# prashantpandeygit/solvingpapers

Hardware: AMD Instinct MI355X
Metric: training tokens/sec, LLaMA3-8B-shape bf16 (higher is better)
Workload: dtype bf16; 1 GPU; model=llama3_8b, global_batch=4, seq_len=8192, parallelism=dp1, micro_batch=1, grad_accum=4, params=8030261248

## Files before the change

### csrc/include/act_common.h

```cpp
#pragma once
#include "spa_common.h"

namespace spa {

enum ActKind : int { RELU = 0, LEAKY = 1, PRELU = 2, ELU = 3, GELU_TANH = 4, GELU_ERF = 5, SILU = 6,
                     SIGMOID = 7, TANH = 8, IDENT = 9 };

__device__ __forceinline__ float act_f(int kind, float x, float a) {
  switch (kind) {
    case RELU: return x > 0.f ? x : 0.f;
    case LEAKY:
    case PRELU: return x > 0.f ? x : a * x;
    case ELU: return x > 0.f ? x : a * (__expf(x) - 1.f);
    case GELU_TANH: {
      const float k0 = 0.7978845608028654f, k1 = 0.044715f;
      const float u = k0 * (x + k1 * x * x * x);
      return 0.5f * x * (1.f + tanhf(u));
    }
    case GELU_ERF: return 0.5f * x * (1.f + erff(x * 0.7071067811865476f));
    case SILU: return x / (1.f + __expf(-x));
    case SIGMOID: return 1.f / (1.f + __expf(-x));
    case TANH: return tanhf(x);
    default: return x;
  }
}
__device__ __forceinline__ float act_df(int kind, float x, float a) {
  switch (kind) {
    case RELU: return x > 0.f ? 1.f : 0.f;
    case LEAKY:
    case PRELU: return x > 0.f ? 1.f : a;
    case ELU: return x > 0.f ? 1.f : a * __expf(x);
    case GELU_TANH: {
      const float k0 = 0.7978845608028654f, k1 = 0.044715f;
      const float u = k0 * (x + k1 * x * x * x);
      const float th = tanhf(u);
      return 0.5f * (1.f + th) + 0.5f * x * (1.f - th * th) * k0 * (1.f + 3.f * k1 * x * x);
    }
    case GELU_ERF: {
      const float cdf = 0.5f * (1.f + erff(x * 0.7071067811865476f));
      const float pdf = 0.3989422804014327f * __expf(-0.5f * x * x);
      return cdf + x * pdf;
    }
    case SILU: {
      const float s = 1.f / (1.f + __expf(-x));
      return s * (1.f + x * (1.f - s));
    }
    case SIGMOID: {
      const float s = 1.f / (1.f + __expf(-x));
      return s * (1.f - s);
    }
    case TANH: {
      const float t = tanhf(x);
      return 1.f - t * t;
    }
    default: return 1.f;
  }
}

}
```

### csrc/kernels/activation.hip

```cpp
#include "act_common.h"

namespace spa {

template <typename T, int KIND>
__global__ __launch_bounds__(256) void act_fwd_kernel(const T* __restrict__ x, T* __restrict__ y, long n, float a) {
  const long nv = n / 8;
  for (long i = blockIdx.x * 256L + threadIdx.x; i < nv; i += (long)gridDim.x * 256) {
    float v[8];
    load8(x + i * 8, v);
#pragma unroll
    for (int k = 0; k < 8; ++k) v[k] = act_f(KIND, v[k], a);
    store8(y + i * 8, v);
  }
  for (long i = nv * 8 + blockIdx.x * 256L + threadIdx.x; i < n; i += (long)gridDim.x * 256)
    y[i] = (T)act_f(KIND, (float)x[i], a);
}
template <typename T, int KIND>
__global__ __launch_bounds__(256) void act_bwd_kernel(const T* __restrict__ dy, const T* __restrict__ x,
                                                      T* __restrict__ dx, long n, float a) {
  const long nv = n / 8;
  for (long i = blockIdx.x * 256L + threadIdx.x; i < nv; i += (long)gridDim.x * 256) {
    float v[8], g[8];
    load8(x + i * 8, v);
    load8(dy + i * 8, g);
#pragma unroll
    for (int k = 0; k < 8; ++k) v[k] = g[k] * act_df(KIND, v[k], a);
    store8(dx + i * 8, v);
  }
  for (long i = nv * 8 + blockIdx.x * 256L + threadIdx.x; i < n; i += (long)gridDim.x * 256)
    dx[i] = (T)((float)dy[i] * act_df(KIND, (float)x[i], a));
}

template <typename T, int KIND>
__global__ __launch_bounds__(256) void glu_fwd_kernel(const T* __restrict__ gu, T* __restrict__ y, long M, int F) {
  const int fv = F / 8;
  const long nv = M * fv;
  for (long i = blockIdx.x * 256L + threadIdx.x; i < nv; i += (long)gridDim.x * 256) {
    const long m = i / fv;
    const int f = (i % fv) * 8;
    float g[8], u[8];
    load8(gu + m * 2 * F + f, g);
    load8(gu + m * 2 * F + F + f, u);
#pragma unroll
    for (int k = 0; k < 8; ++k) g[k] = act_f(KIND, g[k], 0.f) * u[k];
    store8(y + m * F + f, g);
  }
}
template <typename T, int KIND>
__global__ __launch_bounds__(256) void glu_bwd_kernel(const T* __restrict__ dy, const T* __restrict__ gu,
                                                      T* __restrict__ dgu, long M, int F) {
  const int fv = F / 8;
  const long nv = M * fv;
  for (long i = blockIdx.x * 256L + threadIdx.x; i < nv; i += (long)gridDim.x * 256) {
    const long m = i / fv;
    const int f = (i % fv) * 8;
    float g[8], u[8], d[8], dg[8], du[8];
    load8(gu + m * 2 * F + f, g);
    load8(gu + m * 2 * F + F + f, u);
    load8(dy + m * F + f, d);
#pragma unroll
    for (int k = 0; k < 8; ++k) {
      du[k] = d[k] * act_f(KIND, g[k], 0.f);
      dg[k] = d[k] * u[k] * act_df(KIND, g[k], 0.f);
    }
    store8(dgu + m * 2 * F + f, dg);
    store8(dgu + m * 2 * F + F + f, du);
  }
}

#ifndef GLU_T_TT_BWD
#define GLU_T_TT_BWD 128
#endif
#ifndef GLU_T_TT_FWD
#define GLU_T_TT_FWD 64
#endif
template <int KIND>
__global__ __launch_bounds__(256) void glu_bwd_t_kernel(const bf16* __restrict__ dy, const bf16* __restrict__ gu,
                                                        bf16* __restrict__ dgu, bf16* __restrict__ dgut, int M, int F) {
  constexpr int TT = GLU_T_TT_BWD, TF = 128, LD = TF + 8, CT = TT / 8;
  __shared__ __attribute__((aligned(16))) bf16 tile[2][TT * LD];
  const int r0 = blockIdx.y * TT, f0 = blockIdx.x * TF;
  auto soff = [](int r, int c16) { return r * LD + 8 * (c16 ^ ((r >> 3) & 7)); };
#pragma unroll
  for (int c = 0; c < TT / 16; ++c) {
    const int idx = threadIdx.x + 256 * c, r = idx >> 4, ch = idx & 15;
    const int m = r0 + r, f = f0 + ch * 8;
    float g[8], u[8], d[8], dg[8], du[8];
    const bool ok = m < M && f < F;
    if (ok) {
      load8(gu + (long)m * 2 * F + f, g);
      load8(gu + (long)m * 2 * F + F + f, u);
      load8(dy + (long)m * F + f, d);
    }
#pragma unroll
    for (int k = 0; k < 8; ++k) {
      du[k] = ok ? d[k] * act_f(KIND, g[k], 0.f) : 0.f;
      dg[k] = ok ? d[k] * u[k] * act_df(KIND, g[k], 0.f) : 0.f;
    }
    if (ok) {
      store8(dgu + (long)m * 2 * F + f, dg);
      store8(dgu + (long)m * 2 * F + F + f, du);
    }
    bf16x8 a8, b8;
#pragma unroll
    for (int k = 0; k < 8; ++k) { a8[k] = (bf16)dg[k]; b8[k] = (bf16)du[k]; }
    *reinterpret_cast<bf16x8*>(&tile[0][soff(r, ch)]) = a8;
    *reinterpret_cast<bf16x8*>(&tile[1][soff(r, ch)]) = b8;
  }
  __syncthreads();
#pragma unroll
  for (int c = 0; c < CT / 4; ++c) {
    const int idx = threadIdx.x + 256 * c, h = idx / (32 * CT), jq = (idx / CT) & 31, ch = idx % CT;
    uint2 rw[8];
#pragma unroll
    for (int e = 0; e < 8; ++e) {
      const int r = ch * 8 + e;
      rw[e] = *reinterpret_cast<const uint2*>(&tile[h][soff(r, jq >> 1) + 4 * (jq & 1)]);
    }
    const int m = r0 + ch * 8;
    if (m < M) {
#pragma unroll
      for (int q = 0; q < 4; ++q) {
        const int f = f0 + 4 * jq + q;
        if (f < F) {
          const unsigned sel = (q & 1) ? 0x07060302u : 0x05040100u;
          unsigned w[8];
#pragma unroll
          for (int e = 0; e < 8; ++e) w[e] = (q >> 1) ? rw[e].y : rw[e].x;
          uint4 o;
          o.x = __builtin_amdgcn_perm(w[1], w[0], sel);
          o.y = __builtin_amdgcn_perm(w[3], w[2], sel);
          o.z = __builtin_amdgcn_perm(w[5], w[4], sel);
          o.w = __builtin_amdgcn_perm(w[7], w[6], sel);
          *reinterpret_cast<uint4*>(dgut + (long)(h * F + f) * M + m) = o;
        }
      }
    }
  }
}

template <int KIND>
__global__ __launch_bounds__(256) void glu_fwd_t_kernel(const bf16* __restrict__ gu, bf16* __restrict__ y,
                                                        bf16* __restrict__ yt, int M, int F) {
  constexpr int TT = GLU_T_TT_FWD, TF = 128, LD = TF + 8, CT = TT / 8;
  __shared__ __attribute__((aligned(16))) bf16 tile[TT * LD];
  const int r0 = blockIdx.y * TT, f0 = blockIdx.x * TF;
  auto soff = [](int r, int c16) { return r * LD + 8 * (c16 ^ ((r >> 3) & 7)); };
#pragma unroll
  for (int c = 0; c < TT / 16; ++c) {
    const int idx = threadIdx.x + 256 * c, r = idx >> 4, ch = idx & 15;
    const int m = r0 + r, f = f0 + ch * 8;
    float g[8], u[8];
    const bool ok = m < M && f < F;
    if (ok) {
      load8(gu + (long)m * 2 * F + f, g);
      load8(gu + (long)m * 2 * F + F + f, u);
    }
#pragma unroll
    for (int k = 0; k < 8; ++k) g[k] = ok ? act_f(KIND, g[k], 0.f) * u[k] : 0.f;
    if (ok) store8(y + (long)m * F + f, g);
    bf16x8 a8;
#pragma unroll
    for (int k = 0; k < 8; ++k) a8[k] = (bf16)g[k];
    *reinterpret_cast<bf16x8*>(&tile[soff(r, ch)]) = a8;
  }
  __syncthreads();
#pragma unroll
  for (int c = 0; c < CT / 8; ++c) {
  const int idx = threadIdx.x + 256 * c, jq = idx / CT, ch = idx % CT;
  uint2 rw[8];
#pragma unroll
  for (int e = 0; e < 8; ++e) rw[e] = *reinterpret_cast<const uint2*>(&tile[soff(ch * 8 + e, jq >> 1) + 4 * (jq & 1)]);
  const int m = r0 + ch * 8;
  if (m < M) {
#pragma unroll
    for (int q = 0; q < 4; ++q) {
      const int f = f0 + 4 * jq + q;
      if (f < F) {
        const unsigned sel = (q & 1) ? 0x07060302u : 0x05040100u;
        unsigned w[8];
#pragma unroll
        for (int e = 0; e < 8; ++e) w[e] = (q >> 1) ? rw[e].y : rw[e].x;
        uint4 o;
        o.x = __builtin_amdgcn_perm(w[1], w[0], sel);
        o.y = __builtin_amdgcn_perm(w[3], w[2], sel);
        o.z = __builtin_amdgcn_perm(w[5], w[4], sel);
        o.w = __builtin_amdgcn_perm(w[7], w[6], sel);
        *reinterpret_cast<uint4*>(yt + (long)f * M + m) = o;
      }
    }
  }
  }
}

template <int KIND>
__global__ __launch_bounds__(256) void act_bwd_colsum_kernel(const bf16* __restrict__ dy, const bf16* __restrict__ u,
                                                             bf16* __restrict__ du, float* __restrict__ part,
                                                             long R, int N, long rpb, float a) {
  __shared__ __attribute__((aligned(16))) float red[8][256];
  const int cl = threadIdx.x & 31, rg = threadIdx.x >> 5;
  const int c0 = blockIdx.x * 256 + cl * 8;
  const long r0 = (long)blockIdx.y * rpb, r1 = min(R, r0 + rpb);
  float acc[8] = {0.f, 0.f, 0.f, 0.f, 0.f, 0.f, 0.f, 0.f};
  auto one = [&](const float* g, const float* x, long r) {
    float d[8];
#pragma unroll
    for (int k = 0; k < 8; ++k) {
      d[k] = g[k] * act_df(KIND, x[k], a);
    }
    store8(du + r * N + c0, d);
#pragma unroll
    for (int k = 0; k < 8; ++k) acc[k] += (float)(bf16)d[k];
  };
  if (c0 < N) {
    long r = r0 + rg;
    for (; r + 24 < r1; r += 32) {
      float g[4][8], x[4][8];
#pragma unroll
      for (int k = 0; k < 4; ++k) {
        load8(dy + (r + 8 * k) * N + c0, g[k]);
        load8(u + (r + 8 * k) * N + c0, x[k]);
      }
#pragma unroll
      for (int k = 0; k < 4; ++k) one(g[k], x[k], r + 8 * k);
    }
    for (; r < r1; r += 8) {
      float g0[8], x0[8];
      load8(dy + r * N + c0, g0);
      load8(u + r * N + c0, x0);
      one(g0, x0, r);
    }
  }
  *reinterpret_cast<float4*>(&red[rg][cl * 8]) = make_float4(acc[0], acc[1], acc[2], acc[3]);
  *reinterpret_cast<float4*>(&red[rg][cl * 8 + 4]) = make_float4(acc[4], acc[5], acc[6], acc[7]);
  __syncthreads();
  const int c = blockIdx.x * 256 + threadIdx.x;
  if (c < N) {
    float t = 0.f;
#pragma unroll
    for (int g = 0; g < 8; ++g) t += red[g][threadIdx.x];
    part[(long)blockIdx.y * N + c] = t;
  }
}

static int ew_grid(long n) { return (int)std::max<long>(1, std::min<long>((n + 255) / 256, 8192)); }

#define ACT_SWITCH(KIND, ...)                                         \
  switch (KIND) {                                                     \
    case RELU: { constexpr int K_ = RELU; __VA_ARGS__; break; }       \
    case LEAKY: { constexpr int K_ = LEAKY; __VA_ARGS__; break; }     \
    case PRELU: { constexpr int K_ = PRELU; __VA_ARGS__; break; }     \
    case ELU: { constexpr int K_ = ELU; __VA_ARGS__; break; }         \
    case GELU_TANH: { constexpr int K_ = GELU_TANH; __VA_ARGS__; break; } \
    case GELU_ERF: { constexpr int K_ = GELU_ERF; __VA_ARGS__; break; }   \
    case SILU: { constexpr int K_ = SILU; __VA_ARGS__; break; }       \
    case SIGMOID: { constexpr int K_ = SIGMOID; __VA_ARGS__; break; } \
    case TANH: { constexpr int K_ = TANH; __VA_ARGS__; break; }       \
    default: TORCH_CHECK(false, "unknown activation kind");          \
  }

#define DTYPE_SWITCH(ST, ...)                                                       \
  if (ST == at::kBFloat16) { using T_ = bf16; __VA_ARGS__; }                        \
  else if (ST == at::kFloat) { using T_ = float; __VA_ARGS__; }                     \
  else TORCH_CHECK(false, "only bf16 / fp32 supported");

at::Tensor act_fwd(const at::Tensor& x_, int64_t kind, double alpha) {
  SPA_CHECK_CUDA(x_);
  auto x = dense(x_);
  auto y = at::empty_like(x);
  const long n = x.numel();
  if (n == 0) return y;
  DeviceGuard g(x.device());
  auto st = stream();
  DTYPE_SWITCH(x.scalar_type(), ACT_SWITCH(kind, act_fwd_kernel<T_, K_><<<ew_grid(n / 8 + 1), 256, 0, st>>>(
                                                    (const T_*)x.data_ptr(), (T_*)y.data_ptr(), n, (float)alpha)));
  SPA_LAUNCH_CHECK();
  return y;
}
at::Tensor act_bwd(const at::Tensor& dy_, const at::Tensor& x_, int64_t kind, double alpha) {
  auto x = dense(x_);
  auto dy = dense_like(dy_, x);
  TORCH_CHECK(dy.scalar_type() == x.scalar_type() && dy.numel() == x.numel());
  auto dx = at::empty_like(x);
  const long n = x.numel();
  if (n == 0) return dx;
  DeviceGuard g(x.device());
  auto st = stream();
  DTYPE_SWITCH(x.scalar_type(),
               ACT_SWITCH(kind, act_bwd_kernel<T_, K_><<<ew_grid(n / 8 + 1), 256, 0, st>>>(
                                    (const T_*)dy.data_ptr(), (const T_*)x.data_ptr(), (T_*)dx.data_ptr(), n,
                                    (float)alpha)));
  SPA_LAUNCH_CHECK();
  return dx;
}
std::vector<at::Tensor> act_bwd_colsum(const at::Tensor& dy, const at::Tensor& u, int64_t kind, double alpha) {
  SPA_CHECK_CUDA(u);
  TORCH_CHECK(u.dim() == 2 && u.scalar_type() == at::kBFloat16 && u.is_contiguous(), "act_bwd_colsum: [R, N] bf16");
  TORCH_CHECK(dy.sizes() == u.sizes() && dy.scalar_type() == at::kBFloat16 && dy.is_contiguous(),
              "act_bwd_colsum: dy must match u");
  const long R = u.size(0);
  const int N = u.size(1);
  TORCH_CHECK(N % 8 == 0 && (uintptr_t)u.data_ptr() % 16 == 0 && (uintptr_t)dy.data_ptr() % 16 == 0,
              "act_bwd_colsum: 16-byte rows");
  DeviceGuard g(u.device());
  auto du = at::empty_like(u);
  auto opts = u.options().dtype(at::kFloat);
  if (N == 0) return {du, at::empty({0}, opts)};
  if (R == 0) return {du, at::zeros({N}, opts)};
  auto st = stream();
  const int nx = cdiv(N, 256);
  const long want = std::max<long>(1, std::min<long>(cdiv(2048, nx), cdiv(R, 128)));
  const long rpb = (R + want - 1) / want;
  const int P = (int)cdiv(R, rpb);
  auto part = at::empty({P, N}, opts);
  ACT_SWITCH(kind, act_bwd_colsum_kernel<K_><<<dim3(nx, P), 256, 0, st>>>(
                       (const bf16*)dy.data_ptr(), (const bf16*)u.data_ptr(), (bf16*)du.data_ptr(),
                       part.data_ptr<float>(), R, N, rpb, (float)alpha));
  SPA_LAUNCH_CHECK();
  return {du, reduce_col_parts(part)};
}
at::Tensor glu_fwd(const at::Tensor& gu_, int64_t kind) {
  SPA_CHECK_CUDA(gu_);
  auto gu = gu_.contiguous();
  const int F2 = gu.size(-1);
  TORCH_CHECK(F2 % 16 == 0, "glu: last dim must be 2F with F % 8 == 0");
  const int F = F2 / 2;
  const long M = gu.numel() / F2;
  auto sizes = gu.sizes().vec();
  sizes.back() = F;
  auto y = at::empty(sizes, gu.options());
  if (M == 0) return y;
  DeviceGuard g(gu.device());
  auto st = stream();
  DTYPE_SWITCH(gu.scalar_type(), ACT_SWITCH(kind, glu_fwd_kernel<T_, K_><<<ew_grid(M * F / 8), 256, 0, st>>>(
                                                     (const T_*)gu.data_ptr(), (T_*)y.data_ptr(), M, F)));
  SPA_LAUNCH_CHECK();
  return y;
}
at::Tensor glu_bwd(const at::Tensor& dy_, const at::Tensor& gu_, int64_t kind) {
  auto gu = gu_.contiguous();
  auto dy = dy_.contiguous();
  const int F2 = gu.size(-1), F = F2 / 2;
  const long M = gu.numel() / F2;
  TORCH_CHECK(dy.numel() == M * F && dy.scalar_type() == gu.scalar_type());
  auto dgu = at::empty_like(gu);
  if (M == 0) return dgu;
  DeviceGuard g(gu.device());
  auto st = stream();
  DTYPE_SWITCH(gu.scalar_type(),
               ACT_SWITCH(kind, glu_bwd_kernel<T_, K_><<<ew_grid(M * F / 8), 256, 0, st>>>(
                                    (const T_*)dy.data_ptr(), (const T_*)gu.data_ptr(), (T_*)dgu.data_ptr(), M, F)));
  SPA_LAUNCH_CHECK();
  return dgu;
}

std::vector<at::Tensor> glu_fwd_t(const at::Tensor& gu_, int64_t kind) {
  auto gu = gu_.contiguous();
  TORCH_CHECK(gu.scalar_type() == at::kBFloat16, "glu_fwd_t: bf16");
  const int F2 = gu.size(-1), F = F2 / 2;
  const long M = gu.numel() / F2;
  TORCH_CHECK(F2 % 16 == 0 && M % 8 == 0 && M < (1L << 31), "glu_fwd_t: M % 8, F % 8");
  auto sizes = gu.sizes().vec();
  sizes.back() = F;
  auto y = at::empty(sizes, gu.options());
  auto yt = at::empty({F, M}, gu.options());
  if (M == 0) return {y, yt};
  DeviceGuard g(gu.device());
  const dim3 grid(cdiv(F, 128), (int)cdiv(M, (long)GLU_T_TT_FWD));
  ACT_SWITCH(kind, glu_fwd_t_kernel<K_><<<grid, 256, 0, stream()>>>((const bf16*)gu.data_ptr(), (bf16*)y.data_ptr(),
                                                                      (bf16*)yt.data_ptr(), (int)M, F));
  SPA_LAUNCH_CHECK();
  return {y, yt};
}

std::vector<at::Tensor> glu_bwd_t(const at::Tensor& dy_, const at::Tensor& gu_, int64_t kind) {
  auto gu = gu_.contiguous();
  auto dy = dy_.contiguous();
  TORCH_CHECK(gu.scalar_type() == at::kBFloat16 && dy.scalar_type() == at::kBFloat16, "glu_bwd_t: bf16");
  const int F2 = gu.size(-1), F = F2 / 2;
  const long M = gu.numel() / F2;
  TORCH_CHECK(dy.numel() == M * F, "glu_bwd_t: dy must be [.., F]");
  TORCH_CHECK(M % 8 == 0 && F % 8 == 0 && M < (1L << 31) && (long)F2 * M < (1L << 40), "glu_bwd_t: M, F % 8");
  auto dgu = at::empty_like(gu);
  auto dgut = at::empty({F2, M}, gu.options());
  if (M == 0) return {dgu, dgut};
  DeviceGuard g(gu.device());
  const dim3 grid(cdiv(F, 128), (int)cdiv(M, (long)GLU_T_TT_BWD));
  ACT_SWITCH(kind, glu_bwd_t_kernel<K_><<<grid, 256, 0, stream()>>>(
                       (const bf16*)dy.data_ptr(), (const bf16*)gu.data_ptr(), (bf16*)dgu.data_ptr(),
                       (bf16*)dgut.data_ptr(), (int)M, F));
  SPA_LAUNCH_CHECK();
  return {dgu, dgut};
}

}

TORCH_LIBRARY_FRAGMENT(spa, m) {
  m.def("glu_bwd_t(Tensor dy, Tensor gu, int kind) -> Tensor[]");
  m.def("glu_fwd_t(Tensor gu, int kind) -> Tensor[]");
  m.def("act_fwd(Tensor x, int kind, float alpha) -> Tensor");
  m.def("act_bwd(Tensor dy, Tensor x, int kind, float alpha) -> Tensor");
  m.def("act_bwd_colsum(Tensor dy, Tensor u, int kind, float alpha) -> Tensor[]");
  m.def("glu_fwd(Tensor gu, int kind) -> Tensor");
  m.def("glu_bwd(Tensor dy, Tensor gu, int kind) -> Tensor");
}
TORCH_LIBRARY_IMPL(spa, CUDA, m) {
  m.impl("glu_bwd_t", &spa::glu_bwd_t);
  m.impl("glu_fwd_t", &spa::glu_fwd_t);
  m.impl("act_fwd", &spa::act_fwd);
  m.impl("act_bwd", &spa::act_bwd);
  m.impl("act_bwd_colsum", &spa::act_bwd_colsum);
  m.impl("glu_fwd", &spa::glu_fwd);
  m.impl("glu_bwd", &spa::glu_bwd);
}
```

### solvingpapers_amd/ops/linear.py

```python
from __future__ import annotations

import os
import weakref

import torch

from ..utils.grad import commit
from . import _ext
from .layout import bias_grad, wgrad

GEMV = os.environ.get("SPA_GEMV", "1") != "0"
GEMV_MAX_ROWS = 4

DGRAD_WT = os.environ.get("SPA_DGRAD_WT", "1") != "0"
DGRAD_WT_MIN_NUMEL = int(os.environ.get("SPA_DGRAD_WT_MIN", str(1 << 18)))
_WT_CACHE: dict = {}


def invalidate_weight_caches():
    from .moe import bump_weight_epoch
    bump_weight_epoch()


def transposed_weight(w: torch.Tensor):
    if not (DGRAD_WT and w.is_cuda and w.dtype == torch.bfloat16 and w.dim() == 2 and w.is_contiguous()
            and w.numel() >= DGRAD_WT_MIN_NUMEL and w.shape[0] % 8 == 0 and w.shape[1] % 8 == 0
            and w.data_ptr() % 16 == 0):
        return None
    from .layout import transpose2d
    from .moe import _WEIGHT_EPOCH
    if torch.cuda.is_current_stream_capturing():
        with torch.no_grad():
            return transpose2d(w)
    key = (_WEIGHT_EPOCH[0], w._version, w.data_ptr())
    hit = _WT_CACHE.get(id(w))
    if hit is not None and hit[2]() is not w:
        hit = None
    if hit is not None and hit[0] == key:
        return hit[1]
    with torch.no_grad():
        wt = transpose2d(w)
    if hit is None:
        weakref.finalize(w, _WT_CACHE.pop, id(w), None)
    _WT_CACHE[id(w)] = (key, wt, weakref.ref(w))
    return wt


def dgrad(dy2: torch.Tensor, w: torch.Tensor) -> torch.Tensor:
    wt = transposed_weight(w)
    return torch.mm(dy2, w) if wt is None else torch.mm(dy2, wt.t())


def _commit_bias(b, s):
    def _b(out, acc):
        if out is None:
            return s.to(b.dtype)
        if acc:
            out.add_(s.to(out.dtype))
        else:
            out.copy_(s)
    return commit(b, _b)


class _LinearFn(torch.autograd.Function):
    @staticmethod
    def forward(ctx, x, w, b):
        ctx.w, ctx.b = w, b
        ctx.save_for_backward(x)
        x2 = x.reshape(-1, x.shape[-1])
        if b is not None:
            y = torch.addmm(b, x2, w.t())
        else:
            y = torch.mm(x2, w.t())
        return torch.ops.aten._unsafe_view(y, (*x.shape[:-1], w.shape[0]))

    @staticmethod
    def backward(ctx, dy):
        (x,) = ctx.saved_tensors
        w, b = ctx.w, ctx.b
        dy2 = dy.reshape(-1, dy.shape[-1])
        x2 = x.reshape(-1, x.shape[-1])
        dx = dgrad(dy2, w).view(x.shape) if ctx.needs_input_grad[0] else None
        gw = gb = None
        if ctx.needs_input_grad[1]:
            def _w(out, acc):
                return wgrad(dy2, x2, out, acc)
            gw = commit(w, _w)
        if b is not None and ctx.needs_input_grad[2]:
            gb = _commit_bias(b, bias_grad(dy2))
        return dx, gw, gb


class _LinearActFn(torch.autograd.Function):

    @staticmethod
    def forward(ctx, x, w, b, kind, alpha):
        x2 = x.reshape(-1, x.shape[-1])
        u = torch.addmm(b, x2, w.t())
        y = _ext.ops().act_fwd(u, kind, alpha)
        ctx.save_for_backward(x, u)
        ctx.w, ctx.b, ctx.kind, ctx.alpha = w, b, kind, alpha
        return torch.ops.aten._unsafe_view(y, (*x.shape[:-1], w.shape[0]))

    @staticmethod
    def backward(ctx, dy):
        x, u = ctx.saved_tensors
        w, b = ctx.w, ctx.b
        dy2 = dy.reshape(-1, dy.shape[-1]).contiguous()
        x2 = x.reshape(-1, x.shape[-1])
        gb = None
        if ctx.needs_input_grad[2]:
            du, s = _ext.ops().act_bwd_colsum(dy2, u, ctx.kind, ctx.alpha)
            gb = _commit_bias(b, s)
        else:
            du = _ext.ops().act_bwd(dy2, u, ctx.kind, ctx.alpha)
        dx = dgrad(du, w).view(x.shape) if ctx.needs_input_grad[0] else None
        gw = None
        if ctx.needs_input_grad[1]:
            def _w(out, acc):
                return wgrad(du, x2, out, acc)
            gw = commit(w, _w)
        return dx, gw, gb, None, None


class _LinearGluFn(torch.autograd.Function):

    @staticmethod
    def forward(ctx, x, w, kind):
        x2 = x.reshape(-1, x.shape[-1])
        h = torch.mm(x2, w.t())
        f = _ext.ops().glu_fwd(h, kind)
        ctx.save_for_backward(x, h)
        ctx.w, ctx.kind = w, kind
        return torch.ops.aten._unsafe_view(f, (*x.shape[:-1], w.shape[0] // 2))

    @staticmethod
    def backward(ctx, df):
        x, h = ctx.saved_tensors
        w = ctx.w
        x2 = x.reshape(-1, x.shape[-1])
        dh, dht = _ext.ops().glu_bwd_t(df.reshape(-1, df.shape[-1]), h, ctx.kind)
        dx = dgrad(dh, w).view(x.shape) if ctx.needs_input_grad[0] else None
        gw = None
        if ctx.needs_input_grad[1]:
            gw = commit(w, lambda out, acc: wgrad(dh, x2, out, acc, dyt=dht))
        return dx, gw, None


def linear_glu(x, w, kind="silu"):
    from .activation import glu
    from .reference import ACT_KINDS
    if _glu_t_mode() >= 1 and _glu_t_ok(x, w):
        return _LinearGluFn.apply(x, w, ACT_KINDS[kind])
    return glu(linear(x, w), kind)


class _SwiGluMLPFn(torch.autograd.Function):

    @staticmethod
    def forward(ctx, x, w13, w2, kind):
        x2 = x.reshape(-1, x.shape[-1])
        h = torch.mm(x2, w13.t())
        f, ft = _ext.ops().glu_fwd_t(h, kind)
        y = torch.mm(f, w2.t())
        ctx.save_for_backward(x, h, ft)
        ctx.w13, ctx.w2, ctx.kind = w13, w2, kind
        return torch.ops.aten._unsafe_view(y, (*x.shape[:-1], w2.shape[0]))

    @staticmethod
    def backward(ctx, dy):
        from .layout import transpose2d
        x, h, ft = ctx.saved_tensors
        w13, w2 = ctx.w13, ctx.w2
        dy2 = dy.reshape(-1, dy.shape[-1]).contiguous()
        x2 = x.reshape(-1, x.shape[-1])
        need = ctx.needs_input_grad
        dx = gw13 = gw2 = None
        if need[2]:
            dyt = transpose2d(dy2)
            gw2 = commit(w2, lambda out, acc: wgrad(dy2, ft.t(), out, acc, x2t=ft, dyt=dyt))
        dh, dht = _ext.ops().glu_bwd_t(dgrad(dy2, w2), h, ctx.kind)
        if need[0]:
            dx = dgrad(dh, w13).view(x.shape)
        if need[1]:
            gw13 = commit(w13, lambda out, acc: wgrad(dh, x2, out, acc, dyt=dht))
        return dx, gw13, gw2, None


def _glu_t_mode() -> int:
    return int(os.environ.get("SPA_GLU_T", "2"))


def _glu_t_ok(x, w) -> bool:
    T = x.numel() // x.shape[-1] if x.shape[-1] else 0
    return (x.is_cuda and x.dtype == torch.bfloat16 and w.dtype == torch.bfloat16 and w.dim() == 2
            and w.shape[0] % 16 == 0 and x.shape[-1] % 8 == 0 and T >= 2048 and T % 8 == 0
            and not torch.cuda.is_current_stream_capturing())


def swiglu_mlp(x, w13, w2, kind="silu"):
    if _glu_t_mode() >= 2 and _glu_t_ok(x, w13) and w2.dtype == torch.bfloat16 and w2.dim() == 2:
        from .reference import ACT_KINDS
        return _SwiGluMLPFn.apply(x, w13, w2, ACT_KINDS[kind])
    return linear(linear_glu(x, w13, kind), w2)


def linear_act(x, w, b, kind="gelu", alpha=None):
    from .activation import act
    from .reference import ACT_KINDS
    if (b is not None and x.is_cuda and x.dtype == torch.bfloat16 and w.dtype == torch.bfloat16
            and w.shape[0] % 8 == 0 and x.shape[-1] % 8 == 0 and x.numel() > 0):
        if alpha is None:
            alpha = 0.01 if kind == "leaky_relu" else (1.0 if kind == "elu" else 0.0)
        return _LinearActFn.apply(x, w, b, ACT_KINDS[kind], float(alpha))
    return act(linear(x, w, b), kind, alpha)


def mlp(x, w1, b1, w2, b2, kind="gelu", alpha=None):
    return linear(linear_act(x, w1, b1, kind, alpha), w2, b2)


def _gemv_ok(x, w, b) -> bool:
    if not (GEMV and b is None and x.is_cuda and x.dtype == torch.bfloat16 and w.dtype == torch.bfloat16):
        return False
    if torch.is_grad_enabled() and (x.requires_grad or w.requires_grad):
        return False
    K = x.shape[-1]
    rows = x.numel() // K if K else 0
    return (1 <= rows <= GEMV_MAX_ROWS and K % 8 == 0 and w.dim() == 2 and w.stride(1) == 1
            and w.stride(0) % 8 == 0 and w.data_ptr() % 16 == 0 and x.stride(-1) == 1
            and x.data_ptr() % 16 == 0)


def _w8_cpu_ok(x, w, b) -> bool:
    if x.is_cuda or b is not None or w.dim() != 2 or not x.is_floating_point():
        return False
    if torch.is_grad_enabled() and (x.requires_grad or w.requires_grad):
        return False
    K = x.shape[-1]
    return 1 <= (x.numel() // K if K else 0) <= GEMV_MAX_ROWS


class _LinearFP8Fn(torch.autograd.Function):

    @staticmethod
    def forward(ctx, x, w, b):
        from .moe import quant_rows_fp8, quant_weight_fp8_rows
        ctx.w, ctx.b = w, b
        ctx.save_for_backward(x)
        x2 = x.reshape(-1, x.shape[-1])
        xq, sx = quant_rows_fp8(x2)
        wq, sw, _, _ = quant_weight_fp8_rows(w)
        y = torch._scaled_mm(xq, wq.t(), sx[:, None], sw[None, :], bias=b, out_dtype=x.dtype)
        return torch.ops.aten._unsafe_view(y, (*x.shape[:-1], w.shape[0]))

    @staticmethod
    def backward(ctx, dy):
        from .moe import quant_rows_fp8, quant_weight_fp8_rows
        (x,) = ctx.saved_tensors
        w, b = ctx.w, ctx.b
        dy2 = dy.reshape(-1, dy.shape[-1]).contiguous()
        x2 = x.reshape(-1, x.shape[-1])
        dx = None
        if ctx.needs_input_grad[0]:
            dq, sd = quant_rows_fp8(dy2)
            _, _, wtq, swt = quant_weight_fp8_rows(w)
            dx = torch._scaled_mm(dq, wtq.t(), sd[:, None], swt[None, :], out_dtype=dy.dtype).view(x.shape)
        gw = gb = None
        if ctx.needs_input_grad[1] and _dense_wgrad_fp8_ok(dy2, x2, w):
            gw = _dense_wgrad_fp8(w, dy2, x2)
        elif ctx.needs_input_grad[1]:
            def _w(out, acc):
                return wgrad(dy2, x2, out, acc)
            gw = commit(w, _w)
        if b is not None and ctx.needs_input_grad[2]:
            gb = _commit_bias(b, bias_grad(dy2))
        return dx, gw, gb


def _dense_wgrad_fp8_ok(dy2, x2, w):
    from .moe import FP8_WGRAD
    return (FP8_WGRAD and dy2.is_cuda and w.dim() == 2 and w.shape[0] % 128 == 0 and w.shape[1] % 128 == 0
            and dy2.shape[0] > 0)


def _dense_wgrad_fp8(w, dy2, x2):
    from .moe import commit_weight_grad_fp8, padded_offsets, quant_t_fp8_seg
    T = dy2.shape[0]
    off = _one_group(T, dy2.device)
    poff, ld = padded_offsets(off), (T + 127) // 128 * 128
    aq, sa = quant_t_fp8_seg(dy2, off, poff, ld)
    bq, sb = quant_t_fp8_seg(x2, off, poff, ld)
    return commit_weight_grad_fp8(w, aq, sa, bq, sb, poff)


_GROUP1: dict = {}


def _one_group(rows, device):
    key = (rows, str(device))
    t = _GROUP1.get(key)
    if t is None:
        t = torch.tensor([0, rows], dtype=torch.int32, device=device)
        if len(_GROUP1) > 512:
            _GROUP1.clear()
        _GROUP1[key] = t
    return t


def _fp8_ok(x, w) -> bool:
    K = x.shape[-1]
    return (x.is_cuda and x.dtype == torch.bfloat16 and w.dtype == torch.bfloat16 and w.dim() == 2
            and w.shape[0] % 16 == 0 and K % 16 == 0 and x.numel() > 0 and (x.numel() // K) % 16 == 0)


def linear(x, w, b=None, fp8=False):
    if getattr(w, "_spa_w8", None) is not None:
        if _gemv_ok(x, w, b):
            from .moe import w8_image
            wq, s = w8_image(w)
            x2 = x.reshape(-1, x.shape[-1])
            if x2.stride(0) % 8:
                x2 = x2.contiguous()
            return _ext.ops().gemv_w8(x2, wq, s).view(*x.shape[:-1], w.shape[0])
        if _w8_cpu_ok(x, w, b):
            from .moe import w8_image
            from .reference import gemv_w8
            wq, s = w8_image(w)
            return gemv_w8(x.reshape(-1, x.shape[-1]), wq, s).to(x.dtype).view(*x.shape[:-1], w.shape[0])
    if fp8 and _fp8_ok(x, w) and not _gemv_ok(x, w, b):
        return _LinearFP8Fn.apply(x, w, b)
    if _gemv_ok(x, w, b):
        x2 = x.reshape(-1, x.shape[-1])
        if x2.stride(0) % 8:
            x2 = x2.contiguous()
        return _ext.ops().gemv(x2, w).view(*x.shape[:-1], w.shape[0])
    return _LinearFn.apply(x, w, b)


_JOINT: dict = {}


def _joint_views(ws):
    w0 = ws[0]
    mgs = [getattr(w, "main_grad", None) for w in ws]
    if any(m is None for m in mgs):
        return None
    ptrs = tuple(w.data_ptr() for w in ws) + tuple(m.data_ptr() for m in mgs)
    key = tuple(id(w) for w in ws)
    hit = _JOINT.get(key)
    if hit is not None and hit[3] == ptrs and all(r() is w for r, w in zip(hit[2], ws)):
        return hit[0], hit[1]
    K = w0.shape[1]
    rows, off_w, off_g = 0, 0, 0
    for w, m in zip(ws, mgs):
        if (w.dim() != 2 or w.shape[1] != K or w.dtype != w0.dtype or not w.is_contiguous()
                or not m.is_contiguous() or m.dtype != mgs[0].dtype or m.shape != w.shape):
            return None
        if w.data_ptr() != w0.data_ptr() + off_w or m.data_ptr() != mgs[0].data_ptr() + off_g:
            return None
        off_w += w.numel() * w.element_size()
        off_g += m.numel() * m.element_size()
        rows += w.shape[0]
    wd, md = w0.detach(), mgs[0]
    if wd.storage_offset() + rows * K > wd.untyped_storage().nbytes() // wd.element_size():
        return None
    W = wd.as_strided((rows, K), (K, 1), wd.storage_offset())
    MG = md.as_strided((rows, K), (K, 1), md.storage_offset())
    if hit is None:
        weakref.finalize(w0, _JOINT.pop, key, None)
    _JOINT[key] = (W, MG, tuple(weakref.ref(w) for w in ws), ptrs)
    return W, MG


class _LinearRowsFn(torch.autograd.Function):

    @staticmethod
    def forward(ctx, x, W, MG, *ws):
        ctx.W, ctx.MG, ctx.ws = W, MG, ws
        ctx.save_for_backward(x)
        x2 = x.reshape(-1, x.shape[-1])
        return torch.ops.aten._unsafe_view(torch.mm(x2, W.t()), (*x.shape[:-1], W.shape[0]))

    @staticmethod
    def backward(ctx, dy):
        from ..utils.grad import _Gen
        (x,) = ctx.saved_tensors
        dy2 = dy.reshape(-1, dy.shape[-1])
        x2 = x.reshape(-1, x.shape[-1])
        dx = dgrad(dy2, ctx.W).view(x.shape) if ctx.needs_input_grad[0] else None
        if any(ctx.needs_input_grad[3:]):
            acc = getattr(ctx.ws[0], "_spa_gen", -1) == _Gen.value
            assert all((getattr(w, "_spa_gen", -1) == _Gen.value) == acc for w in ctx.ws), \
                "linear_rows: weights committed apart within one iteration"
            wgrad(dy2, x2, ctx.MG, acc)
            for w in ctx.ws:
                w._spa_gen = _Gen.value
        return (dx, None, None) + (None,) * len(ctx.ws)


def linear_rows(x, ws):
    jv = _joint_views(ws)
    if jv is not None and not _gemv_ok(x, jv[0], None):
        return _LinearRowsFn.apply(x, jv[0], jv[1], *ws)
    return torch.cat([linear(x, w) for w in ws], dim=-1)


class Linear(torch.nn.Module):

    def __init__(self, in_features, out_features, bias=True, device=None, dtype=None):
        super().__init__()
        self.in_features, self.out_features = in_features, out_features
        self.weight = torch.nn.Parameter(torch.empty(out_features, in_features, device=device, dtype=dtype))
        self.bias = torch.nn.Parameter(torch.empty(out_features, device=device, dtype=dtype)) if bias else None
        self.reset_parameters()

    def reset_parameters(self):
        torch.nn.init.kaiming_uniform_(self.weight, a=5 ** 0.5)
        if self.bias is not None:
            bound = 1 / self.in_features ** 0.5
            torch.nn.init.uniform_(self.bias, -bound, bound)

    def forward(self, x):
        return linear(x, self.weight, self.bias)

    def extra_repr(self):
        return f"in_features={self.in_features}, out_features={self.out_features}, bias={self.bias is not None}"
```

Before: 22880 tokens/s.

## Rework SwiGLU transpose kernels with fast SiLU, edge specialization and smaller tiles

Adds a SiLU path that computes value and derivative together using hardware exp2 and reciprocal intrinsics, and uses it in all GLU kernels. The fused GLU+transpose forward and backward kernels are restructured: all loads are issued up front into registers, interior tiles take a bounds-check-free template specialization, and the backward tile height drops from 128 to 64 rows. The grid-stride GLU kernels replace per-iteration 64-bit division with incremental row/column stepping. On the Python side, the transposed path is skipped when no gradient is needed, avoiding the extra transpose output in inference. The fast SiLU approximation may change results slightly.

```diff
diff --git a/csrc/include/act_common.h b/csrc/include/act_common.h
--- a/csrc/include/act_common.h
+++ b/csrc/include/act_common.h
@@ -57,4 +57,37 @@
   }
 }
 
+__device__ __forceinline__ void silu_vd(float x, float& val, float& der) {
+#pragma clang fp contract(off)
+  const float e = __builtin_amdgcn_exp2f(x * -1.4426950408889634f);
+  const float s = __builtin_amdgcn_rcpf(__builtin_fmaf(e, 0x1p-32f, 0x1p-32f)) * 0x1p-32f;
+  val = x * s;
+  der = __builtin_fmaf(val, 1.f - s, s);
 }
+
+template <int KIND>
+__device__ __forceinline__ float glu_f(float g, float u) {
+  if constexpr (KIND == SILU) {
+#pragma clang fp contract(off)
+    float v, d;
+    silu_vd(g, v, d);
+    return v * u;
+  } else {
+    return act_f(KIND, g, 0.f) * u;
+  }
+}
+template <int KIND>
+__device__ __forceinline__ void glu_df(float g, float u, float d, float& dg, float& du) {
+  if constexpr (KIND == SILU) {
+#pragma clang fp contract(off)
+    float v, s;
+    silu_vd(g, v, s);
+    du = d * v;
+    dg = d * u * s;
+  } else {
+    du = d * act_f(KIND, g, 0.f);
+    dg = d * u * act_df(KIND, g, 0.f);
+  }
+}
+
+}
diff --git a/csrc/kernels/activation.hip b/csrc/kernels/activation.hip
--- a/csrc/kernels/activation.hip
+++ b/csrc/kernels/activation.hip
@@ -34,15 +34,19 @@
 template <typename T, int KIND>
 __global__ __launch_bounds__(256) void glu_fwd_kernel(const T* __restrict__ gu, T* __restrict__ y, long M, int F) {
   const int fv = F / 8;
-  const long nv = M * fv;
-  for (long i = blockIdx.x * 256L + threadIdx.x; i < nv; i += (long)gridDim.x * 256) {
-    const long m = i / fv;
-    const int f = (i % fv) * 8;
+  const long i0 = blockIdx.x * 256L + threadIdx.x, step = (long)gridDim.x * 256;
+  const long sm = step / fv;
+  const int sc = (int)(step - sm * fv);
+  long m = i0 / fv;
+  int c = (int)(i0 - m * fv);
+  for (; m < M; m += sm, c += sc) {
+    if (c >= fv) { c -= fv; ++m; if (m >= M) break; }
+    const int f = c * 8;
     float g[8], u[8];
     load8(gu + m * 2 * F + f, g);
     load8(gu + m * 2 * F + F + f, u);
 #pragma unroll
-    for (int k = 0; k < 8; ++k) g[k] = act_f(KIND, g[k], 0.f) * u[k];
+    for (int k = 0; k < 8; ++k) g[k] = glu_f<KIND>(g[k], u[k]);
     store8(y + m * F + f, g);
   }
 }
@@ -50,147 +54,153 @@
 __global__ __launch_bounds__(256) void glu_bwd_kernel(const T* __restrict__ dy, const T* __restrict__ gu,
                                                       T* __restrict__ dgu, long M, int F) {
   const int fv = F / 8;
-  const long nv = M * fv;
-  for (long i = blockIdx.x * 256L + threadIdx.x; i < nv; i += (long)gridDim.x * 256) {
-    const long m = i / fv;
-    const int f = (i % fv) * 8;
+  const long i0 = blockIdx.x * 256L + threadIdx.x, step = (long)gridDim.x * 256;
+  const long sm = step / fv;
+  const int sc = (int)(step - sm * fv);
+  long m = i0 / fv;
+  int c = (int)(i0 - m * fv);
+  for (; m < M; m += sm, c += sc) {
+    if (c >= fv) { c -= fv; ++m; if (m >= M) break; }
+    const int f = c * 8;
     float g[8], u[8], d[8], dg[8], du[8];
     load8(gu + m * 2 * F + f, g);
     load8(gu + m * 2 * F + F + f, u);
     load8(dy + m * F + f, d);
 #pragma unroll
-    for (int k = 0; k < 8; ++k) {
-      du[k] = d[k] * act_f(KIND, g[k], 0.f);
-      dg[k] = d[k] * u[k] * act_df(KIND, g[k], 0.f);
-    }
+    for (int k = 0; k < 8; ++k) glu_df<KIND>(g[k], u[k], d[k], dg[k], du[k]);
     store8(dgu + m * 2 * F + f, dg);
     store8(dgu + m * 2 * F + F + f, du);
   }
 }
 
-#ifndef GLU_T_TT_BWD
-#define GLU_T_TT_BWD 128
-#endif
-#ifndef GLU_T_TT_FWD
-#define GLU_T_TT_FWD 64
-#endif
+constexpr int GLU_T_TT = 64, GLU_T_TF = 128, GLU_T_LD = GLU_T_TF + 8;
+__device__ __forceinline__ int glu_t_soff(int r, int c16) { return r * GLU_T_LD + 8 * (c16 ^ ((r >> 3) & 7)); }
+
+template <bool EDGE>
+__device__ __forceinline__ void glu_t_store_job(const bf16* tile, bf16* __restrict__ out, int M, int F, int r0,
+                                                int f0, int jq, int ch) {
+  uint2 rw[8];
+#pragma unroll
+  for (int e = 0; e < 8; ++e)
+    rw[e] = *reinterpret_cast<const uint2*>(&tile[glu_t_soff(ch * 8 + e, jq >> 1) + 4 * (jq & 1)]);
+  const int m = r0 + ch * 8;
+  if (EDGE && m >= M) return;
+#pragma unroll
+  for (int q = 0; q < 4; ++q) {
+    const int f = f0 + 4 * jq + q;
+    if (EDGE && f >= F) continue;
+    const unsigned sel = (q & 1) ? 0x07060302u : 0x05040100u;
+    unsigned w[8];
+#pragma unroll
+    for (int e = 0; e < 8; ++e) w[e] = (q >> 1) ? rw[e].y : rw[e].x;
+    uint4 o;
+    o.x = __builtin_amdgcn_perm(w[1], w[0], sel);
+    o.y = __builtin_amdgcn_perm(w[3], w[2], sel);
+    o.z = __builtin_amdgcn_perm(w[5], w[4], sel);
+    o.w = __builtin_amdgcn_perm(w[7], w[6], sel);
+    *reinterpret_cast<uint4*>(out + (long)f * M + m) = o;
+  }
+}
+
+template <int KIND, int TT, bool EDGE>
+__device__ __forceinline__ void glu_bwd_t_tile(const bf16* __restrict__ dy, const bf16* __restrict__ gu,
+                                               bf16* __restrict__ dgu, bf16* __restrict__ dgut, int M, int F,
+                                               int r0, int f0, bf16* tg, bf16* tu) {
+  constexpr int NC = TT / 16, CT = TT / 8;
+  const int rr = threadIdx.x >> 4, ch = threadIdx.x & 15, f = f0 + ch * 8;
+  bf16x8 gr[NC], ur[NC], dr[NC];
+#pragma unroll
+  for (int c = 0; c < NC; ++c) {
+    const int m = r0 + rr + 16 * c;
+    if (!EDGE || (m < M && f < F)) {
+      gr[c] = *reinterpret_cast<const bf16x8*>(gu + (long)m * 2 * F + f);
+      ur[c] = *reinterpret_cast<const bf16x8*>(gu + (long)m * 2 * F + F + f);
+      dr[c] = *reinterpret_cast<const bf16x8*>(dy + (long)m * F + f);
+    } else {
+#pragma unroll
+      for (int k = 0; k < 8; ++k) gr[c][k] = ur[c][k] = dr[c][k] = (bf16)0.f;
+    }
+  }
+#pragma unroll
+  for (int c = 0; c < NC; ++c) {
+    const int r = rr + 16 * c, m = r0 + r;
+    bf16x8 a8, b8;
+#pragma unroll
+    for (int k = 0; k < 8; ++k) {
+      float dg, du;
+      glu_df<KIND>((float)gr[c][k], (float)ur[c][k], (float)dr[c][k], dg, du);
+      a8[k] = (bf16)dg;
+      b8[k] = (bf16)du;
+    }
+    if (!EDGE || (m < M && f < F)) {
+      *reinterpret_cast<bf16x8*>(dgu + (long)m * 2 * F + f) = a8;
+      *reinterpret_cast<bf16x8*>(dgu + (long)m * 2 * F + F + f) = b8;
+    }
+    *reinterpret_cast<bf16x8*>(&tg[glu_t_soff(r, ch)]) = a8;
+    *reinterpret_cast<bf16x8*>(&tu[glu_t_soff(r, ch)]) = b8;
+  }
+  __syncthreads();
+#pragma unroll
+  for (int c = 0; c < CT / 4; ++c) {
+    const int idx = threadIdx.x + 256 * c, h = idx / (32 * CT), jq = (idx / CT) & 31;
+    glu_t_store_job<EDGE>(h ? tu : tg, dgut + (long)h * F * M, M, F, r0, f0, jq, idx % CT);
+  }
+}
 template <int KIND>
 __global__ __launch_bounds__(256) void glu_bwd_t_kernel(const bf16* __restrict__ dy, const bf16* __restrict__ gu,
                                                         bf16* __restrict__ dgu, bf16* __restrict__ dgut, int M, int F) {
-  constexpr int TT = GLU_T_TT_BWD, TF = 128, LD = TF + 8, CT = TT / 8;
-  __shared__ __attribute__((aligned(16))) bf16 tile[2][TT * LD];
-  const int r0 = blockIdx.y * TT, f0 = blockIdx.x * TF;
-  auto soff = [](int r, int c16) { return r * LD + 8 * (c16 ^ ((r >> 3) & 7)); };
-#pragma unroll
-  for (int c = 0; c < TT / 16; ++c) {
-    const int idx = threadIdx.x + 256 * c, r = idx >> 4, ch = idx & 15;
-    const int m = r0 + r, f = f0 + ch * 8;
-    float g[8], u[8], d[8], dg[8], du[8];
-    const bool ok = m < M && f < F;
-    if (ok) {
-      load8(gu + (long)m * 2 * F + f, g);
-      load8(gu + (long)m * 2 * F + F + f, u);
-      load8(dy + (long)m * F + f, d);
-    }
-#pragma unroll
-    for (int k = 0; k < 8; ++k) {
-      du[k] = ok ? d[k] * act_f(KIND, g[k], 0.f) : 0.f;
-      dg[k] = ok ? d[k] * u[k] * act_df(KIND, g[k], 0.f) : 0.f;
-    }
-    if (ok) {
-      store8(dgu + (long)m * 2 * F + f, dg);
-      store8(dgu + (long)m * 2 * F + F + f, du);
-    }
-    bf16x8 a8, b8;
-#pragma unroll
-    for (int k = 0; k < 8; ++k) { a8[k] = (bf16)dg[k]; b8[k] = (bf16)du[k]; }
-    *reinterpret_cast<bf16x8*>(&tile[0][soff(r, ch)]) = a8;
-    *reinterpret_cast<bf16x8*>(&tile[1][soff(r, ch)]) = b8;
+  constexpr int TT = GLU_T_TT;
+  __shared__ __attribute__((aligned(16))) bf16 tile[2][TT * GLU_T_LD];
+  const int r0 = blockIdx.y * TT, f0 = blockIdx.x * GLU_T_TF;
+  if (r0 + TT <= M && f0 + GLU_T_TF <= F)
+    glu_bwd_t_tile<KIND, TT, false>(dy, gu, dgu, dgut, M, F, r0, f0, tile[0], tile[1]);
+  else
+    glu_bwd_t_tile<KIND, TT, true>(dy, gu, dgu, dgut, M, F, r0, f0, tile[0], tile[1]);
+}
+
+template <int KIND, int TT, bool EDGE>
+__device__ __forceinline__ void glu_fwd_t_tile(const bf16* __restrict__ gu, bf16* __restrict__ y,
+                                               bf16* __restrict__ yt, int M, int F, int r0, int f0, bf16* tile) {
+  constexpr int NC = TT / 16, CT = TT / 8;
+  const int rr = threadIdx.x >> 4, ch = threadIdx.x & 15, f = f0 + ch * 8;
+  bf16x8 gr[NC], ur[NC];
+#pragma unroll
+  for (int c = 0; c < NC; ++c) {
+    const int m = r0 + rr + 16 * c;
+    if (!EDGE || (m < M && f < F)) {
+      gr[c] = *reinterpret_cast<const bf16x8*>(gu + (long)m * 2 * F + f);
+      ur[c] = *reinterpret_cast<const bf16x8*>(gu + (long)m * 2 * F + F + f);
+    } else {
+#pragma unroll
+      for (int k = 0; k < 8; ++k) gr[c][k] = ur[c][k] = (bf16)0.f;
+    }
+  }
+#pragma unroll
+  for (int c = 0; c < NC; ++c) {
+    const int r = rr + 16 * c, m = r0 + r;
+    bf16x8 a8;
+#pragma unroll
+    for (int k = 0; k < 8; ++k) a8[k] = (bf16)glu_f<KIND>((float)gr[c][k], (float)ur[c][k]);
+    if (!EDGE || (m < M && f < F)) *reinterpret_cast<bf16x8*>(y + (long)m * F + f) = a8;
+    *reinterpret_cast<bf16x8*>(&tile[glu_t_soff(r, ch)]) = a8;
   }
   __syncthreads();
 #pragma unroll
-  for (int c = 0; c < CT / 4; ++c) {
-    const int idx = threadIdx.x + 256 * c, h = idx / (32 * CT), jq = (idx / CT) & 31, ch = idx % CT;
-    uint2 rw[8];
-#pragma unroll
-    for (int e = 0; e < 8; ++e) {
-      const int r = ch * 8 + e;
-      rw[e] = *reinterpret_cast<const uint2*>(&tile[h][soff(r, jq >> 1) + 4 * (jq & 1)]);
-    }
-    const int m = r0 + ch * 8;
-    if (m < M) {
-#pragma unroll
-      for (int q = 0; q < 4; ++q) {
-        const int f = f0 + 4 * jq + q;
-        if (f < F) {
-          const unsigned sel = (q & 1) ? 0x07060302u : 0x05040100u;
-          unsigned w[8];
-#pragma unroll
-          for (int e = 0; e < 8; ++e) w[e] = (q >> 1) ? rw[e].y : rw[e].x;
-          uint4 o;
-          o.x = __builtin_amdgcn_perm(w[1], w[0], sel);
-          o.y = __builtin_amdgcn_perm(w[3], w[2], sel);
-          o.z = __builtin_amdgcn_perm(w[5], w[4], sel);
-          o.w = __builtin_amdgcn_perm(w[7], w[6], sel);
-          *reinterpret_cast<uint4*>(dgut + (long)(h * F + f) * M + m) = o;
-        }
-      }
-    }
-  }
-}
-
+  for (int c = 0; c < CT / 8; ++c) {
+    const int idx = threadIdx.x + 256 * c;
+    glu_t_store_job<EDGE>(tile, yt, M, F, r0, f0, idx / CT, idx % CT);
+  }
+}
 template <int KIND>
 __global__ __launch_bounds__(256) void glu_fwd_t_kernel(const bf16* __restrict__ gu, bf16* __restrict__ y,
                                                         bf16* __restrict__ yt, int M, int F) {
-  constexpr int TT = GLU_T_TT_FWD, TF = 128, LD = TF + 8, CT = TT / 8;
-  __shared__ __attribute__((aligned(16))) bf16 tile[TT * LD];
-  const int r0 = blockIdx.y * TT, f0 = blockIdx.x * TF;
-  auto soff = [](int r, int c16) { return r * LD + 8 * (c16 ^ ((r >> 3) & 7)); };
-#pragma unroll
-  for (int c = 0; c < TT / 16; ++c) {
-    const int idx = threadIdx.x + 256 * c, r = idx >> 4, ch = idx & 15;
-    const int m = r0 + r, f = f0 + ch * 8;
-    float g[8], u[8];
-    const bool ok = m < M && f < F;
-    if (ok) {
-      load8(gu + (long)m * 2 * F + f, g);
-      load8(gu + (long)m * 2 * F + F + f, u);
-    }
-#pragma unroll
-    for (int k = 0; k < 8; ++k) g[k] = ok ? act_f(KIND, g[k], 0.f) * u[k] : 0.f;
-    if (ok) store8(y + (long)m * F + f, g);
-    bf16x8 a8;
-#pragma unroll
-    for (int k = 0; k < 8; ++k) a8[k] = (bf16)g[k];
-    *reinterpret_cast<bf16x8*>(&tile[soff(r, ch)]) = a8;
-  }
-  __syncthreads();
-#pragma unroll
-  for (int c = 0; c < CT / 8; ++c) {
-  const int idx = threadIdx.x + 256 * c, jq = idx / CT, ch = idx % CT;
-  uint2 rw[8];
-#pragma unroll
-  for (int e = 0; e < 8; ++e) rw[e] = *reinterpret_cast<const uint2*>(&tile[soff(ch * 8 + e, jq >> 1) + 4 * (jq & 1)]);
-  const int m = r0 + ch * 8;
-  if (m < M) {
-#pragma unroll
-    for (int q = 0; q < 4; ++q) {
-      const int f = f0 + 4 * jq + q;
-      if (f < F) {
-        const unsigned sel = (q & 1) ? 0x07060302u : 0x05040100u;
-        unsigned w[8];
-#pragma unroll
-        for (int e = 0; e < 8; ++e) w[e] = (q >> 1) ? rw[e].y : rw[e].x;
-        uint4 o;
-        o.x = __builtin_amdgcn_perm(w[1], w[0], sel);
-        o.y = __builtin_amdgcn_perm(w[3], w[2], sel);
-        o.z = __builtin_amdgcn_perm(w[5], w[4], sel);
-        o.w = __builtin_amdgcn_perm(w[7], w[6], sel);
-        *reinterpret_cast<uint4*>(yt + (long)f * M + m) = o;
-      }
-    }
-  }
-  }
+  constexpr int TT = GLU_T_TT;
+  __shared__ __attribute__((aligned(16))) bf16 tile[TT * GLU_T_LD];
+  const int r0 = blockIdx.y * TT, f0 = blockIdx.x * GLU_T_TF;
+  if (r0 + TT <= M && f0 + GLU_T_TF <= F)
+    glu_fwd_t_tile<KIND, TT, false>(gu, y, yt, M, F, r0, f0, tile);
+  else
+    glu_fwd_t_tile<KIND, TT, true>(gu, y, yt, M, F, r0, f0, tile);
 }
 
 template <int KIND>
@@ -366,7 +376,7 @@
   auto yt = at::empty({F, M}, gu.options());
   if (M == 0) return {y, yt};
   DeviceGuard g(gu.device());
-  const dim3 grid(cdiv(F, 128), (int)cdiv(M, (long)GLU_T_TT_FWD));
+  const dim3 grid(cdiv(F, 128), (int)cdiv(M, (long)GLU_T_TT));
   ACT_SWITCH(kind, glu_fwd_t_kernel<K_><<<grid, 256, 0, stream()>>>((const bf16*)gu.data_ptr(), (bf16*)y.data_ptr(),
                                                                       (bf16*)yt.data_ptr(), (int)M, F));
   SPA_LAUNCH_CHECK();
@@ -385,7 +395,7 @@
   auto dgut = at::empty({F2, M}, gu.options());
   if (M == 0) return {dgu, dgut};
   DeviceGuard g(gu.device());
-  const dim3 grid(cdiv(F, 128), (int)cdiv(M, (long)GLU_T_TT_BWD));
+  const dim3 grid(cdiv(F, 128), (int)cdiv(M, (long)GLU_T_TT));
   ACT_SWITCH(kind, glu_bwd_t_kernel<K_><<<grid, 256, 0, stream()>>>(
                        (const bf16*)dy.data_ptr(), (const bf16*)gu.data_ptr(), (bf16*)dgu.data_ptr(),
                        (bf16*)dgut.data_ptr(), (int)M, F));
diff --git a/solvingpapers_amd/ops/linear.py b/solvingpapers_amd/ops/linear.py
--- a/solvingpapers_amd/ops/linear.py
+++ b/solvingpapers_amd/ops/linear.py
@@ -150,7 +150,7 @@
 def linear_glu(x, w, kind="silu"):
     from .activation import glu
     from .reference import ACT_KINDS
-    if _glu_t_mode() >= 1 and _glu_t_ok(x, w):
+    if _glu_t_mode() >= 1 and _glu_t_ok(x, w) and _needs_grad(x, w):
         return _LinearGluFn.apply(x, w, ACT_KINDS[kind])
     return glu(linear(x, w), kind)
 
@@ -198,8 +198,13 @@
             and not torch.cuda.is_current_stream_capturing())
 
 
+def _needs_grad(*ts) -> bool:
+    return torch.is_grad_enabled() and any(t.requires_grad for t in ts)
+
+
 def swiglu_mlp(x, w13, w2, kind="silu"):
-    if _glu_t_mode() >= 2 and _glu_t_ok(x, w13) and w2.dtype == torch.bfloat16 and w2.dim() == 2:
+    if (_glu_t_mode() >= 2 and _glu_t_ok(x, w13) and w2.dtype == torch.bfloat16 and w2.dim() == 2
+            and _needs_grad(x, w13, w2)):
         from .reference import ACT_KINDS
         return _SwiGluMLPFn.apply(x, w13, w2, ACT_KINDS[kind])
     return linear(linear_glu(x, w13, kind), w2)
```

New measurement: 22920 tokens/s (median of 6 runs). About the same (+0.2%).
